# msaelices/mojo-regex

Hardware: AMD Instinct MI355X
Metric: GB/s input scanned + matches/sec, 1M x 1KiB batch, [a-z]+\d+ DFA (higher is better)
Workload: dtype u8

## Files before the change

### include/mrx_testing.h

```cpp
#ifndef MRX_TESTING_H
#define MRX_TESTING_H

#include <stddef.h>
#include <stdint.h>

#ifdef __cplusplus
extern "C" {
#endif

void mrx_timing_reset(void);
void mrx_timing_enable(int on);
double mrx_timing_scan_ms(int64_t* launches);
const char* mrx_last_kernel_name(void);
void mrx_debug_force_generic(int on);
void mrx_debug_long_text_kernels(int mode);
void mrx_debug_fused_findall(int mode);
void mrx_debug_stream_bits(int on);
void mrx_debug_stream_bits_trace(int64_t* d_trace);
void mrx_debug_dynamic_texts(int mode);
void mrx_debug_split_findall(int on);
void mrx_debug_dense_rows(int mode);
void mrx_debug_tries_always(int on);
void mrx_debug_chain_sub_general(int on);
int mrx_testing_emptywalk_findall(const mrx_handle* h, const uint8_t* text, int len, int32_t* spans, int cap);
void mrx_debug_subs_group(int lanes);
void mrx_debug_litscan_pieces(int mode);
void mrx_debug_multiwalk(int mode);
void mrx_debug_rec_skew(int64_t bytes);
void mrx_debug_rec12(int mode);
int mrx_testing_rec12_roundtrip(int start, int pair, int lane, int before, int32_t out[4]);
void mrx_debug_decode_lean(int mode);
int mrx_debug_last_decode_lean(void);
int mrx_testing_decode_expand(int64_t n, const uint32_t* f_even, const uint32_t* f_odd, const int32_t* start, const int32_t* pb,
                              int fixed_len, int32_t* counts, int32_t* spans);
int mrx_testing_comm_shift(const int64_t* d_prefix, int64_t n_local, const int64_t* d_meta_all, int meta_stride, int rank,
                           int64_t* d_out, int64_t pad_to, void* stream);
int mrx_testing_comm_compact(const int64_t* d_meta_all, int meta_stride, int nranks, const int64_t* d_stage_prefix, int64_t P,
                             const int32_t* d_stage_spans, int64_t cap, int64_t* d_gprefix, int64_t gprefix_cap,
                             int32_t* d_gspans, int64_t gspans_cap, int32_t* d_status, void* stream);
void mrx_debug_set_route(int mode);
struct mrx_set;
int mrx_testing_set_run(const struct mrx_set* s, int op, const uint8_t* text, int len, int32_t* out);
void mrx_debug_filter_form(int form);
void mrx_debug_extract_grid(int workgroups);
void mrx_debug_expand_grid(int workgroups);
void mrx_debug_distinct_hash_mask(uint64_t mask);
void mrx_debug_distinct_grid(int workgroups);
void mrx_debug_sort_small(int max);
void mrx_debug_sort_grid(int workgroups);
int mrx_debug_sort_rounds(void);
void mrx_debug_parse_grid(int workgroups);
void mrx_debug_format_grid(int workgroups);
int mrx_testing_format_one(int32_t kind, int32_t arg, int64_t value_word, uint8_t out[32]);
void mrx_debug_kw_piece(int64_t bytes);
void mrx_debug_kw_tier(int on);
int mrx_debug_kw_host_findall(const uint8_t* entry_data, const int64_t* entry_offsets, int64_t m, uint32_t flags,
                              const uint8_t* data, const int64_t* offsets, int64_t n, int64_t* text_prefix, int32_t* entries,
                              int32_t* spans, int64_t span_cap, int64_t* total, char* describe, size_t describe_cap);
int mrx_debug_kw_host_leftmost(const uint8_t* entry_data, const int64_t* entry_offsets, int64_t m, uint32_t flags, int64_t count,
                               const uint8_t* data, const int64_t* offsets, int64_t n, int64_t* text_prefix, int32_t* entries,
                               int32_t* spans, int64_t span_cap, int64_t* total);
int mrx_debug_kw_host_sub(const uint8_t* entry_data, const int64_t* entry_offsets, int64_t m, uint32_t flags,
                          const uint8_t* repl_data, const int64_t* repl_offsets, int64_t r, int64_t count, const uint8_t* data,
                          const int64_t* offsets, int64_t n, int64_t* out_offsets, uint8_t* out_data, int64_t out_cap,
                          int32_t* nsub, int64_t* totals);
// ... 24 lines not shown
```

### mojo_regex_amd/api.py

```python
from __future__ import annotations

import ctypes as C
import os
from typing import Iterable, List, Optional, Sequence, Tuple

import numpy as np

_HERE = os.path.dirname(os.path.abspath(__file__))
_LIB_NAME = "libmrx_hip.so"
_lib = None

MRX_OK, MRX_E_SYNTAX, MRX_E_UNSUPPORTED, MRX_E_NO_DEVICE, MRX_E_CAPACITY, MRX_E_ARGUMENT = range(6)


class MrxError(RuntimeError):
    """Any failure reported by libmrx_hip.so."""


class RegexSyntaxError(MrxError):
    """The reference's lexer/parser raises on this pattern (same message)."""


class UnsupportedPattern(MrxError):
    """The reference routes this pattern/operation to an engine outside the hot
# ... 74 lines not shown
        "mrx_split_batch": (C.c_int, [H, u8p, i64p, C.c_int64, C.c_int64, i64p, i32p, C.c_int64, C.POINTER(C.c_int64)]),
        "mrx_split_dev": (C.c_int, [H, C.c_void_p, C.c_void_p, C.c_int64, C.c_int64, C.c_void_p, C.c_void_p, C.c_int64,
                                    C.POINTER(C.c_int64), C.c_void_p]),
        "mrx_split_strided_dev": (C.c_int, [H, C.c_void_p, C.c_int64, C.c_void_p, C.c_int32, C.c_int64, C.c_int64, C.c_void_p,
                                            C.c_void_p, C.c_int64, C.POINTER(C.c_int64), C.c_void_p]),
        "mrx_findall_batch": (C.c_int, [H, u8p, i64p, C.c_int64, i64p, i32p, C.c_int64,
                                        C.POINTER(C.c_int64)]),
        "mrx_captures_batch": (C.c_int, [H, u8p, i64p, C.c_int64, i32p]),
        "mrx_sub_batch": (C.c_int, [H, C.c_char_p, C.c_size_t, C.c_int64, u8p, i64p, C.c_int64, i64p,
                                    u8p, C.c_int64, C.POINTER(C.c_int64)]),
        "mrx_timing_reset": (None, []),
        "mrx_timing_enable": (None, [C.c_int]),
        "mrx_timing_scan_ms": (C.c_double, [C.POINTER(C.c_int64)]),
        "mrx_last_kernel_name": (C.c_char_p, []),
        "mrx_debug_force_generic": (None, [C.c_int]),
        "mrx_debug_long_text_kernels": (None, [C.c_int]),
        "mrx_debug_fused_findall": (None, [C.c_int]),
        "mrx_debug_stream_bits": (None, [C.c_int]),
        "mrx_debug_stream_bits_trace": (None, [C.c_void_p]),
        "mrx_debug_dynamic_texts": (None, [C.c_int]),
        "mrx_debug_subs_group": (None, [C.c_int]),
        "mrx_debug_split_findall": (None, [C.c_int]),
        "mrx_debug_dense_rows": (None, [C.c_int]),
        "mrx_debug_tries_always": (None, [C.c_int]),
        "mrx_debug_chain_sub_general": (None, [C.c_int]),
        "mrx_testing_emptywalk_findall": (C.c_int, [H, C.c_char_p, C.c_int, i32p, C.c_int]),
        "mrx_debug_litscan_pieces": (None, [C.c_int]),
        "mrx_debug_multiwalk": (None, [C.c_int]),
        "mrx_debug_rec_skew": (None, [C.c_int64]),
        "mrx_debug_rec12": (None, [C.c_int]),
        "mrx_testing_rec12_roundtrip": (C.c_int, [C.c_int, C.c_int, C.c_int, C.c_int, C.POINTER(C.c_int32)]),
        "mrx_debug_decode_lean": (None, [C.c_int]),
        "mrx_debug_last_decode_lean": (C.c_int, []),
        "mrx_testing_decode_expand": (C.c_int, [C.c_int64, C.c_void_p, C.c_void_p, C.c_void_p, C.c_void_p, C.c_int,
                                                C.c_void_p, C.c_void_p]),
        "mrx_release_scratch": (None, []),
        "mrx_debug_scratch_bytes": (C.c_size_t, []),
        "mrx_debug_scratch_in_use": (C.c_size_t, []),
        "mrx_version": (C.c_char_p, []),
        "mrx_comm_unique_id": (C.c_int, [C.c_void_p]),
        "mrx_comm_init": (C.c_int, [C.c_void_p, C.c_int, C.c_int, C.POINTER(H)]),
        "mrx_comm_free": (None, [H]),
        "mrx_comm_rank": (C.c_int, [H]),
        "mrx_comm_size": (C.c_int, [H]),
        "mrx_comm_spans_staging_bytes": (C.c_size_t, [H, C.c_int64, C.c_int64]),
        "mrx_comm_reserve": (C.c_int, [H, C.c_size_t]),
        "mrx_allgather_fixed": (C.c_int, [H, C.c_void_p, C.c_void_p, C.c_size_t, C.c_void_p]),
        "mrx_allgatherv_rows": (C.c_int, [H, C.c_void_p, C.c_int64, C.c_size_t, C.c_void_p, C.c_int64,
                                          C.POINTER(C.c_int64), C.c_void_p]),
        "mrx_allgatherv_spans": (C.c_int, [H, i64p, C.c_int64, i32p, C.c_int64, C.c_int64, i64p, C.c_int64, i32p,
                                           C.c_int64, C.POINTER(C.c_int64), C.POINTER(C.c_int64), i32p, C.c_void_p]),
        "mrx_testing_comm_shift": (C.c_int, [i64p, C.c_int64, i64p, C.c_int, C.c_int, i64p, C.c_int64, C.c_void_p]),
        "mrx_testing_comm_compact": (C.c_int, [i64p, C.c_int, C.c_int, i64p, C.c_int64, i32p, C.c_int64, i64p, C.c_int64,
                                               i32p, C.c_int64, i32p, C.c_void_p]),
        "mrx_set_compile": (C.c_int, [C.POINTER(C.c_char_p), C.POINTER(C.c_size_t), C.c_int32, C.c_uint32, C.POINTER(H)]),
        "mrx_set_free": (None, [H]),
        "mrx_set_size": (C.c_int32, [H]),
        "mrx_set_describe": (C.c_size_t, [H, C.c_char_p, C.c_size_t]),
        "mrx_set_search_dev": (C.c_int, [H, u8p, i64p, C.c_int64, i32p, i32p, C.c_void_p]),
        "mrx_set_search_strided_dev": (C.c_int, [H, u8p, C.c_int64, i32p, C.c_int32, C.c_int64, i32p, i32p, C.c_void_p]),
        "mrx_set_count_dev": (C.c_int, [H, u8p, i64p, C.c_int64, i32p, C.c_void_p]),
        "mrx_set_count_strided_dev": (C.c_int, [H, u8p, C.c_int64, i32p, C.c_int32, C.c_int64, i32p, C.c_void_p]),
        "mrx_set_matches_dev": (C.c_int, [H, u8p, i64p, C.c_int64, i64p, C.c_void_p]),
        "mrx_set_matches_strided_dev": (C.c_int, [H, u8p, C.c_int64, i32p, C.c_int32, C.c_int64, i64p, C.c_void_p]),
        "mrx_set_findall_dev": (C.c_int, [H, u8p, i64p, C.c_int64, i64p, i32p, i32p, C.c_int64, C.POINTER(C.c_int64),
                                          C.c_void_p]),
# ... 225 lines not shown
    "mrx_gather_spans_dev", "mrx_gather_spans_strided_dev", "mrx_gather_spans_batch",
    "mrx_extract_dev", "mrx_extract_known_dev", "mrx_extract_strided_dev", "mrx_extract_batch",
    "mrx_expand_spans_dev", "mrx_expand_spans_strided_dev", "mrx_expand_spans_batch",
    "mrx_expand_dev", "mrx_expand_strided_dev", "mrx_expand_batch",
    "mrx_distinct_dev", "mrx_distinct_known_dev", "mrx_distinct_strided_dev", "mrx_distinct_batch",
    "mrx_dict_build_dev", "mrx_dict_build_strided_dev", "mrx_dict_free", "mrx_dict_size", "mrx_dict_distinct",
    "mrx_dict_lookup_dev", "mrx_dict_lookup_strided_dev", "mrx_dict_filter_dev", "mrx_dict_filter_known_dev",
    "mrx_dict_filter_strided_dev", "mrx_dict_lookup_batch",
    "mrx_sort_dev", "mrx_sort_known_dev", "mrx_sort_strided_dev", "mrx_sort_batch",
    "mrx_take_dev", "mrx_take_known_dev", "mrx_take_strided_dev", "mrx_take_batch",
    "mrx_parse_dev", "mrx_parse_strided_dev", "mrx_parse_spans_dev", "mrx_parse_spans_strided_dev", "mrx_parse_batch",
    "mrx_format_dev", "mrx_format_batch",
    "mrx_kw_build", "mrx_kw_build_dev", "mrx_kw_free", "mrx_kw_size", "mrx_kw_distinct", "mrx_kw_describe",
    "mrx_kw_contains_dev", "mrx_kw_contains_strided_dev", "mrx_kw_count_dev", "mrx_kw_count_strided_dev",
    "mrx_kw_findall_dev", "mrx_kw_findall_known_dev", "mrx_kw_findall_strided_dev", "mrx_kw_filter_dev",
    "mrx_kw_filter_known_dev", "mrx_kw_filter_strided_dev", "mrx_kw_findall_batch",
    "mrx_kw_leftmost_dev", "mrx_kw_leftmost_known_dev", "mrx_kw_leftmost_strided_dev", "mrx_kw_leftmost_batch",
    "mrx_kw_sub_dev", "mrx_kw_sub_known_dev", "mrx_kw_sub_strided_dev", "mrx_kw_sub_batch",
    "mrx_lines_dev", "mrx_lines_known_dev", "mrx_lines_strided_dev", "mrx_lines_batch",
    "mrx_fields_dev", "mrx_fields_known_dev", "mrx_fields_strided_dev", "mrx_fields_batch",
    "mrx_translate_dev", "mrx_translate_known_dev", "mrx_translate_strided_dev", "mrx_translate_batch",
    "mrx_strip_dev", "mrx_strip_known_dev", "mrx_strip_strided_dev", "mrx_strip_batch",
]
TESTING_SYMBOLS = [
    "mrx_timing_reset", "mrx_timing_enable", "mrx_timing_scan_ms", "mrx_last_kernel_name",
    "mrx_debug_force_generic", "mrx_debug_long_text_kernels", "mrx_debug_scratch_bytes",
    "mrx_debug_scratch_in_use",
    "mrx_debug_fused_findall", "mrx_debug_stream_bits", "mrx_debug_stream_bits_trace", "mrx_debug_dynamic_texts", "mrx_debug_subs_group",
    "mrx_debug_split_findall", "mrx_debug_dense_rows", "mrx_debug_tries_always", "mrx_debug_chain_sub_general", "mrx_testing_emptywalk_findall", "mrx_debug_litscan_pieces", "mrx_debug_multiwalk", "mrx_debug_rec_skew", "mrx_testing_comm_shift", "mrx_testing_comm_compact",
    "mrx_debug_set_route", "mrx_testing_set_run", "mrx_debug_filter_form", "mrx_debug_extract_grid",
    "mrx_debug_expand_grid", "mrx_debug_distinct_hash_mask", "mrx_debug_distinct_grid",
    "mrx_debug_sort_small", "mrx_debug_sort_grid", "mrx_debug_sort_rounds", "mrx_debug_parse_grid",
    "mrx_debug_decode_lean", "mrx_debug_last_decode_lean", "mrx_testing_decode_expand",
    "mrx_debug_format_grid", "mrx_testing_format_one",
    "mrx_debug_kw_piece", "mrx_debug_kw_tier", "mrx_debug_kw_host_findall",
    "mrx_debug_kw_host_leftmost", "mrx_debug_kw_host_sub",
    "mrx_debug_lines_piece", "mrx_debug_lines_syncs", "mrx_debug_lines_host",
    "mrx_debug_fields_group", "mrx_debug_fields_grid", "mrx_debug_fields_host",
    "mrx_debug_translate_piece", "mrx_debug_translate_syncs", "mrx_debug_translate_host",
    "mrx_debug_strip_host",
]
TESTING_SYMBOLS_NUMBERED = ["mrx_debug_rec12", "mrx_testing_rec12_roundtrip"]
COMM_SYMBOLS = [
    "mrx_comm_unique_id", "mrx_comm_init", "mrx_comm_free", "mrx_comm_rank", "mrx_comm_size",
    "mrx_comm_spans_staging_bytes", "mrx_comm_reserve",
    "mrx_allgather_fixed", "mrx_allgatherv_rows", "mrx_allgatherv_spans",
]


def _b(x) -> bytes:
    if isinstance(x, str):
        return x.encode("utf-8")
    return bytes(x)


def _check(rc: int):
    if rc == MRX_OK:
        return
    msg = load_library().mrx_last_error().decode("utf-8", "replace")
    if rc == MRX_E_SYNTAX:
        raise RegexSyntaxError(msg)
    if rc == MRX_E_UNSUPPORTED:
        raise UnsupportedPattern(msg)
    raise MrxError("mrx error %d: %s" % (rc, msg))


# ... 1897 lines not shown
```

### mojo_regex_amd/csrc/mrx_kernels.hip

```cpp
#include <hip/hip_runtime.h>
#include <atomic>
#include <map>
#include <type_traits>
#include <unordered_map>
#include <chrono>

#include <cstdio>
#include <cstdlib>
#include <cstring>
#include <mutex>
#include <string>
#include <vector>

#include "../../include/mrx.h"
#include "../../include/mrx_testing.h"
#include "mrx_device.hpp"
#include "mrx_host_batch.hpp"
#include "mrx_internal.hpp"
#include "mrx_lookback.hpp"
#include "mrx_rec12.hpp"
#include "mrx_decode_bits.hpp"

using namespace mrx;

namespace {

constexpr int kBlock = 256;

struct Layout : TextBatch {
  Layout() = default;
  Layout(const TextBatch& b) : TextBatch(b) {}
  int32_t split = 0;
  int32_t wide_slots = 0;
  const int32_t* vlen = nullptr;
  const uint32_t* vskip = nullptr;
  const int32_t* vbase = nullptr;
  const int2* pre = nullptr;
  const uint32_t* bm = nullptr;
  const int32_t* bm_cnt = nullptr;
  __host__ __device__ __forceinline__ int64_t bm_row(int64_t i) const {
    return 4 * (offsets ? (offsets[i] >> 7) + 2 * i : i * ((stride >> 7) + 2));
  }
  __device__ __forceinline__ int64_t slot_row(int64_t i, int* cap) const {
    if (offsets) {
// ... 1573 lines not shown
    base = fused_lookback(fz.ctrl, w, nw, lane);
    if (base < 0) {
    } else
    if (total_spans > 3 * tile_cap) {
      fused_fill_tile<REC32, true>(wave_recs, wrec, my_rel, 0, base, tile, tile_bytes, fz.spans, fz.span_cap, fixed_len, lane);
    } else {
      for (int tb = 0; tb < total_spans; tb += tile_cap) {
        fused_fill_tile<REC32, false>(wave_recs, wrec, my_rel, tb, 0, tile, tile_bytes, fz.spans, fz.span_cap, fixed_len, lane);
        fused_store_tile<REC32>(tile, total_spans - tb < tile_cap ? total_spans - tb : tile_cap, base + tb, fz.spans,
                                fz.span_cap, lane);
      }
    }
  }
  const int64_t my_text = (w << 6) + lane;
  if (base < 0) {
    if (lane == 0) { fz.prefix[n] = -1; *fz.total_out = -1; }
    return;
  }
  if (my_text < n) fz.prefix[my_text] = base + my_rel;
  if (my_text == n - 1) { fz.prefix[n] = base + incl; *fz.total_out = base + incl; }
}

template <int MODE, int CH, int AUTO, int CSR, int VIRT = 0, int REC32 = 0>
#ifndef MRX_FUSED_WAVES
#define MRX_FUSED_WAVES 4
#endif
__global__ __launch_bounds__(64 * kStreamWaves, (MODE == ST_FUSED ? MRX_FUSED_WAVES : 1)) void k_stream_findall(
    DevPlan p, const uint8_t* __restrict__ blob, const uint8_t* __restrict__ data, int64_t stride,
    const int32_t* __restrict__ lens, int32_t common_len, const int64_t* __restrict__ offsets,
    int64_t n, int32_t* __restrict__ counts,
    int32_t* __restrict__ wave_nrecs, EvRec* __restrict__ recs, int64_t rec_row,
    int32_t* __restrict__ out_s, int32_t* __restrict__ out_e,
    const int32_t* __restrict__ vlen = nullptr, const uint32_t* __restrict__ vskip = nullptr,
    const FusedArgs* __restrict__ fzp = nullptr) {
#define fz (*fzp)
  constexpr bool RECS = MODE == ST_RECORDS || MODE == ST_FUSED;
  constexpr bool ROWS = MODE == ST_ROWS;
  static_assert(!(MODE == ST_FUSED && VIRT), "pieces of long texts keep the three-launch form");
  static_assert(!ROWS || (!CSR && !VIRT && !REC32), "event rows: texts at a fixed aligned pitch");
  constexpr bool REC12 = REC32 == 2;
  static_assert(!REC12 || (MODE == ST_RECORDS && !CSR && !VIRT), "12-byte records: the three-launch form at a fixed aligned pitch");
  constexpr int kChunk = CH;
  constexpr int kRowPitch = CH + 16;
  constexpr int LPR = CH / 16;
  constexpr int RPI = 64 / LPR;
  constexpr int NL = 64 / RPI;
  __shared__ __align__(16) uint8_t tiles[kStreamWaves][64 * kRowPitch];
  __shared__ __align__(16) uint16_t col_lds[256];
  __shared__ __align__(16) uint16_t col32_lds[AUTO == 5 ? 256 : 2];
  static_assert(AUTO != 5 || MODE != ST_FIRST, "the anchored automaton has no code-column form");
  __shared__ __align__(16) uint4 pmask[17];
  if (threadIdx.x < 17) {
    const int x = threadIdx.x;
    uint32_t w[4];
    for (int j = 0; j < 4; ++j) {
      const int nb = x - 4 * j;
      w[j] = nb <= 0 ? 0u : nb >= 4 ? 0xFFFFFFFFu : ((1u << (8 * nb)) - 1u);
    }
    pmask[x] = make_uint4(w[0], w[1], w[2], w[3]);
  }
  __shared__ unsigned long long blk_ticket[4];
  if (MODE == ST_FUSED && threadIdx.x == 0) {
    blk_ticket[1] = blk_ticket[2] = blk_ticket[3] = 0ull;
    blk_ticket[0] = (1ull << 32) | (uint32_t)__hip_atomic_fetch_add(fz.ctrl, (unsigned long long)kStreamWaves, __ATOMIC_RELAXED,
                                                                    __HIP_MEMORY_SCOPE_AGENT);
  }
  const bool use_fill = AUTO == 5 || (MODE != ST_FIRST && p.st_reset_byte >= 0 && !(MODE == ST_COUNT && (AUTO == 2 || AUTO == 3)));
  const uint32_t fillw = (uint32_t)(p.st_reset_byte & 0xFF) * 0x01010101u;
  extern __shared__ __align__(16) uint8_t stg_lds[];
  if (AUTO == 5) {
    const uint16_t* src = (const uint16_t*)(blob + p.off_stcol32);
    for (int i = threadIdx.x; i < 256; i += blockDim.x) col32_lds[i] = src[i];
  } else if (AUTO == 1) {
    const uint16_t* src = (const uint16_t*)(blob + (MODE == ST_FIRST ? p.off_fa_col : p.off_stcol));
    for (int i = threadIdx.x; i < 256; i += blockDim.x) col_lds[i] = src[i];
  } else if (AUTO == 3) {
    const uint32_t* src = (const uint32_t*)(blob + (MODE == ST_FIRST ? p.off_fa_col : p.off_stcol));
    uint32_t* dst = (uint32_t*)stg_lds;
    for (int i = threadIdx.x; i < 512; i += blockDim.x) dst[i] = src[i];
  } else {
    const uint32_t* src = (const uint32_t*)(blob + (MODE == ST_FIRST ? p.off_fa_cls : p.off_stg_cls));
    uint32_t* dst = (uint32_t*)stg_lds;
    const int words = (MODE == ST_FIRST ? p.fa_bytes : p.stg_bytes) >> 2;
    for (int i = threadIdx.x; i < words; i += blockDim.x) dst[i] = src[i];
  }
  __syncthreads();
  const uint64_t* col64_lds = (const uint64_t*)stg_lds;
  const uint8_t* cls_lds = stg_lds;
  const uint16_t* tr_lds = (const uint16_t*)(stg_lds + (MODE == ST_FIRST ? p.off_fa_trans - p.off_fa_cls
                                                                        : p.off_stg_trans - p.off_stg_cls));
  const uint8_t* acc_lds = stg_lds + (p.off_stg_acc - p.off_stg_cls);
  const uint32_t* pair_lds = (const uint32_t*)(stg_lds + (p.off_stg_pair - p.off_stg_cls));
  const uint32_t fa_dead = AUTO == 2 ? (uint32_t)p.fa_nstates << p.fa_cshift
                                     : (uint32_t)p.fa_nstates * (AUTO == 1 ? 4u : 8u);
  const int lane = threadIdx.x & 63;
  const int wave = threadIdx.x >> 6;
  uint8_t* tile = tiles[wave];
  const int64_t nwaves_total = (n + 63) >> 6;
  const uint32_t accmask = p.st_accept_mask;
  const int seg = lane % LPR;
  const int rsub = lane / LPR;

  unsigned long long tk_next = 0ull;
  bool tk_asked = false;
  uint32_t round = 0;
  bool pend = false;
  int64_t pend_w = 0;
  int pend_cnt = 0, pend_wrec = 0, pend_half = 0, half = 0;
  for (int64_t w = (int64_t)blockIdx.x * kStreamWaves + wave;; w += (int64_t)gridDim.x * kStreamWaves) {
    if (MODE == ST_FUSED) {
      unsigned long long tv;
      while (true) {
        tv = *(volatile unsigned long long*)&blk_ticket[round & 3u];
        if ((uint32_t)(tv >> 32) == round + 1u) break;
        __builtin_amdgcn_s_sleep(1);
      }
      const int64_t first = (int64_t)__builtin_amdgcn_readfirstlane((uint32_t)tv);
      w = first + wave;
      tk_asked = wave == 0 && first < nwaves_total;
      if (tk_asked) {
        if (lane == 0)
          tk_next = __hip_atomic_fetch_add(fz.ctrl, (unsigned long long)kStreamWaves, __ATOMIC_RELAXED, __HIP_MEMORY_SCOPE_AGENT);
        asm volatile("" ::: "memory");
      } else if (wave == 0 && lane == 0) {
        blk_ticket[(round + 1u) & 3u] = ((unsigned long long)(round + 2u) << 32) | (uint32_t)nwaves_total;
      }
      ++round;
    }
    if (w >= nwaves_total) break;
    const int64_t base_text = w << 6;
    const int64_t my_text = base_text + lane;
    const bool live = my_text < n;
    int my_len, mis = 0;
    if (CSR) {
      int64_t o0;
      if (offsets) {
        o0 = live ? offsets[my_text] : 0;
        my_len = live ? (VIRT ? vlen[my_text] : (int)(offsets[my_text + 1] - o0)) : 0;
      } else {
        o0 = my_text * stride;
        my_len = live ? (lens ? lens[my_text] : common_len) : 0;
      }
      const uintptr_t addr = my_len > 0 ? (uintptr_t)(data + o0) : (uintptr_t)blob;
      constexpr uintptr_t kFrameMask = MODE == ST_FIRST ? 15 : 127;
      mis = my_len > 0 ? (int)(addr & kFrameMask) : 0;
      const uintptr_t rb = addr & ~kFrameMask;
      *(uint4*)(tile + lane * kRowPitch + CH) =
          make_uint4((uint32_t)rb, (uint32_t)((uint64_t)rb >> 32), (uint32_t)(mis + my_len), 0u);
      __builtin_amdgcn_fence(__ATOMIC_RELEASE, "wavefront");
      __builtin_amdgcn_wave_barrier();
      __builtin_amdgcn_fence(__ATOMIC_ACQUIRE, "wavefront");
    } else {
      my_len = live ? (lens ? lens[my_text] : common_len) : 0;
    }
    const uint32_t vsk = (VIRT && live) ? vskip[my_text] : 0u;
    const int skip = (int)(vsk & 0x7FFFFFFFu);
    const int flen = mis + my_len;
    int max_len = flen;
    for (int off = 32; off > 0; off >>= 1) max_len = max(max_len, __shfl_xor(max_len, off));

    const uint8_t* wbase = data + base_text * stride;
    const int64_t rows_here = n - base_text < 64 ? n - base_text : 64;
    uint32_t roff[NL];
#pragma unroll
    for (int j = 0; j < NL; ++j) {
      int r = RPI * j + rsub;
      if (r >= rows_here) r = (int)rows_here - 1;
      roff[j] = (uint32_t)(r * stride) + seg * 16;
    }
#define MRX_LOAD_CHUNK(CB)                                                       \
    do {                                                                         \
      uint32_t cb_ = (uint32_t)(CB);                                             \
      if (!CSR && (int64_t)cb_ + seg * 16 >= stride) cb_ = (uint32_t)0 - (uint32_t)(seg * 16); \
      _Pragma("unroll") for (int j_ = 0; j_ < NL; ++j_)                          \
        if (MODE != ST_FIRST || !((skip_rows >> (RPI * j_ + rsub)) & 1ull)) {     \
          if (CSR) {                                                             \
            const uint4 rs_ = *(const uint4*)(tile + (RPI * j_ + rsub) * kRowPitch + CH); \
            uint32_t fo_ = cb_ + seg * 16;                                       \
            if (fo_ >= rs_.z) fo_ = 0;   \
            v[j_] = MRX_LDG((const uint4*)((const uint8_t*)(((uint64_t)rs_.y << 32) | rs_.x) + fo_)); \
          } else {                                                               \
            v[j_] = MRX_LDG((const uint4*)(wbase + (roff[j_] + cb_)));                   \
          }                                                                      \
        }                                                                        \
    } while (0)
    uint64_t skip_rows = 0;

    uint32_t q4 = 0;
    uint32_t q_codes = 0;
    int start = 0;
    int cnt = 0;
    int wrec = 0;
    bool done = !live;
    int res_s = -1, res_e = (MODE == ST_FIRST && live && p.fa_start_acc) ? 0 : -1;
    EvRec* wave_recs = (MODE == ST_RECORDS)
        ? recs + ((CSR && offsets) ? rec_region_start(offsets[base_text], w) : base_text * rec_row)
        : (MODE == ST_FUSED) ? recs + (((int64_t)blockIdx.x * kStreamWaves + wave) * 2 + half) * fz.rec_cap : nullptr;
    uint32_t* const wave_recs12 = REC12 ? (uint32_t*)recs + 3 * (base_text * rec_row) : nullptr;

    if (MODE == ST_FIRST) {
      uint4 pv = make_uint4(0, 0, 0, 0);
      if (live && my_len > 0) {
        if (CSR) pv = *(const uint4*)(((uintptr_t)(data + (offsets ? offsets[my_text] : my_text * stride))) & ~(uintptr_t)15);
        else pv = *(const uint4*)(data + my_text * stride);
      }
      const uint32_t pw[4] = {pv.x, pv.y, pv.z, pv.w};
      uint32_t pq = 0, pF = 0;
#pragma unroll
      for (int k = 0; k < 16; ++k) {
        const uint32_t b = (pw[k >> 2] >> ((k & 3) * 8)) & 0xFFu;
        const bool outside = k < mis || k >= flen;
        uint32_t e;
        if (AUTO == 2) {
          e = tr_lds[pq + cls_lds[b]];
          if (outside) e = pq << 2;
          pq = e >> 2;
        } else if (AUTO == 1) {
          e = (uint32_t)col_lds[b] >> pq;
          if (outside) e = pq;
          pq = e & 0xCu;
        } else {
          e = (uint32_t)(col64_lds[b] >> pq);
          if (outside) e = pq;
          pq = e & 0x38u;
        }
        pF = __builtin_amdgcn_alignbit(e, pF, 2);
      }
      const uint32_t pem = pF & 0xAAAAAAAAu;
      if (__all(!live || pq == fa_dead || flen <= 16)) {
        if (live) {
          int e_ = pem ? ((31 - __builtin_clz(pem)) >> 1) + 1 - mis : (p.fa_start_acc ? 0 : -1);
          if (AUTO == 2 && p.off_fa_end >= 0 && stg_lds[(p.off_fa_end - p.off_fa_cls) + (pq >> p.fa_cshift)]) e_ = my_len;
          out_s[my_text] = e_ >= 0 ? 0 : -1;
          out_e[my_text] = e_;
        }
        continue;
      }
    }
    uint4 v[NL];
#pragma unroll
    for (int j = 0; j < NL; ++j) v[j] = make_uint4(0, 0, 0, 0);
    if (max_len > 0) MRX_LOAD_CHUNK(0);
    uint8_t* wr = tile + rsub * kRowPitch + seg * 16;
    uint4 rowacc[ROWS ? 8 : 1];
    for (int cbase = 0; cbase < max_len; cbase += kChunk) {
#pragma unroll
      for (int j = 0; j < NL; ++j) *(uint4*)(wr + j * RPI * kRowPitch) = v[j];
      __builtin_amdgcn_fence(__ATOMIC_RELEASE, "wavefront");
      __builtin_amdgcn_wave_barrier();
      __builtin_amdgcn_fence(__ATOMIC_ACQUIRE, "wavefront");
      if (MODE == ST_SEARCH) { if (__all(done)) break; }
      if (MODE == ST_FIRST) {
        skip_rows = __ballot(done || cbase + kChunk >= flen);
        if (__all(done)) break;
      }
      if (MODE == ST_FUSED && tk_asked) {
        const uint32_t nf = __builtin_amdgcn_readfirstlane((uint32_t)tk_next);
        if (lane == 0) blk_ticket[round & 3u] = ((unsigned long long)(round + 1u) << 32) | nf;
        tk_asked = false;
      }
      if (!(MRX_ABLATE & 2))
      if (cbase + kChunk < max_len) MRX_LOAD_CHUNK(cbase + kChunk);

      const int lim = flen - cbase;
      const int lo = mis - cbase;
      const bool all_inside = __all(lim >= kChunk && lo <= 0);
      const bool full = all_inside || use_fill;
      uint32_t F_even = 0, meta_even = 0, sp_even = 0;
      uint2 rowbuf[ROWS ? kChunk / 32 : 1];
#pragma unroll
      for (int g = 0; g < kChunk / 16; ++g) {
        const uint4 wv = *(const uint4*)(tile + lane * kRowPitch + g * 16);
        uint32_t words[4] = {wv.x, wv.y, wv.z, wv.w};
        if (use_fill && !all_inside) {
          const int limf = (VIRT && !(vsk >> 31)) ? 0x3FFFFFFF : lim;
          const int a = min(max(lo - g * 16, 0), 16), b = min(max(limf - g * 16, 0), 16);
          const uint4 pa = pmask[a], pb = pmask[b > a ? b : a];
          const uint32_t m[4] = {pb.x & ~pa.x, pb.y & ~pa.y, pb.z & ~pa.z, pb.w & ~pa.w};
#pragma unroll
          for (int j = 0; j < 4; ++j) words[j] = (words[j] & m[j]) | (fillw & ~m[j]);
        }
        uint32_t F = 0;
        if (AUTO == 4) {
          uint32_t cc[16], pi[8];
#pragma unroll
          for (int k = 0; k < 16; ++k)
            cc[k] = cls_lds[(words[k >> 2] >> ((k & 3) * 8)) & 0xFFu];
#pragma unroll
          for (int k = 0; k < 8; ++k) pi[k] = (cc[2 * k] << p.st_cshift) | cc[2 * k + 1];
#pragma unroll
          for (int k = 0; k < 8; ++k) {
            const uint32_t e = pair_lds[q4 + pi[k]];
            q4 = e >> 4;
            F = __builtin_amdgcn_alignbit(e, F, 4);
          }
// ... 189 lines not shown
        for (int off = 32; off > 0; off >>= 1) wt += __shfl_xor(wt, off);
        if (lane == 0) wave_nrecs[nwaves_total + w] = wt;
      }
      if (MODE == ST_FIRST) {
        if (live) {
          if (AUTO == 2 && p.off_fa_end >= 0 && stg_lds[(p.off_fa_end - p.off_fa_cls) + (q4 >> p.fa_cshift)]) res_e = my_len;
          out_s[my_text] = res_e >= 0 ? 0 : -1;
          out_e[my_text] = res_e;
        }
      } else if (MODE == ST_SEARCH) {
        if (live) {
          if (!done && tail) { res_s = p.st_fixed_len > 0 ? my_len - p.st_fixed_len : start; res_e = my_len; }
          out_s[my_text] = res_s;
          out_e[my_text] = res_e;
        }
      } else if (MODE == ST_FUSED) {
        int wt = live ? cnt : 0;
        for (int off = 32; off > 0; off >>= 1) wt += __shfl_xor(wt, off);
        fused_publish(fz.ctrl, w, nwaves_total, (uint32_t)wt, lane);
        if (pend)
          fused_finish<REC32 != 0>(fz, recs + (((int64_t)blockIdx.x * kStreamWaves + wave) * 2 + pend_half) * fz.rec_cap,
                                   pend_w, nwaves_total, n, pend_cnt, pend_wrec, tile, 64 * kRowPitch, p.st_fixed_len, lane);
        pend = true; pend_w = w; pend_cnt = live ? cnt : 0; pend_wrec = wrec; pend_half = half;
        half ^= 1;
      } else {
        if (live) counts[my_text] = cnt;
      }
    }
  }
  if (MODE == ST_FUSED && pend)
    fused_finish<REC32 != 0>(fz, recs + (((int64_t)blockIdx.x * kStreamWaves + wave) * 2 + pend_half) * fz.rec_cap,
                             pend_w, nwaves_total, n, pend_cnt, pend_wrec, tile, 64 * kRowPitch, p.st_fixed_len, lane);
#undef MRX_LOAD_CHUNK
#undef fz
}

#ifndef MRX_DYN_TEXTS
#define MRX_DYN_TEXTS 256
#endif
constexpr int kDynTexts = MRX_DYN_TEXTS;
constexpr int kDynShift = kDynTexts <= 256 ? 24 : kDynTexts <= 512 ? 23 : 22;
constexpr uint32_t kDynBeforeMask = (1u << kDynShift) - 1u;
static_assert(kDynTexts % 64 == 0 && kDynTexts <= 1024, "task size");
__host__ __device__ inline int64_t rec_region_dyn(int64_t first_off, int64_t w) { return (first_off >> 4) + 4 * kDynTexts * w; }

template <int MODE, int AUTO, int REC32>
__global__ __launch_bounds__(64 * kStreamWaves) void k_stream_dyn(
    DevPlan p, const uint8_t* __restrict__ blob, const uint8_t* __restrict__ data, const int64_t* __restrict__ offsets,
    const int32_t* __restrict__ vlen, int64_t n, int32_t* __restrict__ counts, int32_t* __restrict__ wave_nrecs,
    EvRec* __restrict__ recs, int32_t* __restrict__ out_s, int32_t* __restrict__ out_e) {
  static_assert(MODE == ST_RECORDS || MODE == ST_COUNT || MODE == ST_SEARCH, "search modes only");
#ifndef MRX_DYN_CH
#define MRX_DYN_CH 128
#endif
  constexpr int CH = MRX_DYN_CH, kRowPitch = CH + 16, LPR = CH / 16, RPI = 64 / LPR, NL = 64 / RPI;
  __shared__ __align__(16) uint8_t tiles[kStreamWaves][64 * kRowPitch];
  __shared__ __align__(16) uint16_t col_lds[256];
  __shared__ __align__(16) uint4 pmask[17];
  __shared__ uint16_t perm_all[kStreamWaves][kDynTexts];
  __shared__ int hist_all[kStreamWaves][32];
  if (threadIdx.x < 17) {
    const int x = threadIdx.x;
    uint32_t w[4];
    for (int j = 0; j < 4; ++j) {
      const int nb = x - 4 * j;
      w[j] = nb <= 0 ? 0u : nb >= 4 ? 0xFFFFFFFFu : ((1u << (8 * nb)) - 1u);
// ... 2237 lines not shown
  }
  HIP_TRY(hipGetLastError());
  tm.stop();
  return MRX_OK;
}

std::atomic<int> g_fused{0};
std::atomic<int64_t> g_rec_skew{0};
std::atomic<int> g_fused_bpc{0};
int64_t fused_grid_cap() {
  const int bpc = g_fused_bpc.load() > 0 ? g_fused_bpc.load() : 4;
  return (int64_t)(grid_cap() / 8) * bpc;
}
constexpr int64_t kFusedMinTaskBytes = 32768;
bool anchored_at_zero(const mrx_handle* h) {
  const DevPlan& p = h->hp.dev;
  return !g_force_generic && (p.flags & PF_START_ANCHOR) && !(p.flags & PF_PURE_LITERAL) &&
         (!(p.flags & PF_END_ANCHOR) || p.off_fa_end >= 0) &&
         p.kind == PLAN_DFA && p.fa_bytes > 0 && !(p.flags & (PF_EXACT_LITERAL | PF_PREFILTER)) && h->hp.why_no_search.empty();
}
constexpr int64_t kStreamMaxText = int64_t(1) << 26;
bool stream_text_too_long(int64_t max_text) { return max_text >= kStreamMaxText; }
bool stream_layout_ok(const Layout&, int64_t n) { return n > 0; }
bool strided_fast(const Layout& lay) {
  return !lay.offsets && (lay.stride % 16 == 0) && (((uintptr_t)lay.data) % 16 == 0) &&
         lay.stride * 64 < (int64_t(1) << 31);
}

static bool code_columns_on() {
  static const bool on = [] { const char* e = getenv("MRX_NO_CODE_COLUMNS"); return !(e && e[0] == '1'); }();
  return on;
}

template <int MODE>
void launch_stream(const mrx_handle* h, const Layout& lay, int64_t n, int32_t* d_counts, int32_t* d_nrecs,
                   EvRec* d_recs, int64_t rec_row, int32_t* d_s, int32_t* d_e, hipStream_t s,
                   const int32_t* d_vlen = nullptr, const uint32_t* d_vskip = nullptr, int rec32 = 0,
                   const FusedArgs* fused = nullptr, int fused_grid = 0) {
  const DevPlan& p = h->hp.dev;
  const int g = MODE == ST_FUSED ? fused_grid : wave_grid(n, kStreamWaves);
  const FusedArgs* fzv = fused;
  const dim3 grid((unsigned)g), block(64 * kStreamWaves);
  const int kind = MODE == ST_FIRST ? p.fa_kind : p.st_kind;
  const bool table = kind == 2;
  const bool wide = kind == 3;
  const bool pairs = MODE != ST_FIRST && (table || wide) && p.off_stg_pair >= 0 && g_pair_tables;
  const size_t lds = pairs ? (size_t)p.stg_bytes
                           : wide ? 2048 : !table ? 0 : (size_t)(MODE == ST_FIRST ? p.fa_bytes : p.stg_bytes);
#define MRX_LAUNCH_R(AUTO, CSR, R32)                                                              \
  hipLaunchKernelGGL((k_stream_findall<MODE, (AUTO == 2 ? MRX_STREAM_CHUNK_TABLE : MRX_STREAM_CHUNK), AUTO, CSR, 0, R32>), grid, block, lds, s, p, \
                     H_BLOB(h), lay.data, lay.stride, lay.lens, lay.len, lay.offsets, n, d_counts, \
                     d_nrecs, d_recs, rec_row, d_s, d_e, (const int32_t*)nullptr, (const uint32_t*)nullptr, fzv)
#define MRX_LAUNCH(AUTO, CSR)                                                                     \
  do {                                                                                            \
    if constexpr (MODE == ST_RECORDS && CSR == 0) {                                               \
      if (rec32 == 2) { MRX_LAUNCH_R(AUTO, CSR, 2); break; }                                      \
    }                                                                                             \
    if constexpr (MODE == ST_RECORDS || MODE == ST_FUSED) {                                       \
      if (rec32) MRX_LAUNCH_R(AUTO, CSR, 1); else MRX_LAUNCH_R(AUTO, CSR, 0);                     \
    } else MRX_LAUNCH_R(AUTO, CSR, 0);                                                            \
  } while (0)
  if (d_vlen) {
    if constexpr (MODE == ST_RECORDS || MODE == ST_COUNT || MODE == ST_SEARCH || MODE == ST_FIRST) {
#define MRX_LAUNCH_V(AUTO)                                                                        \
  hipLaunchKernelGGL((k_stream_findall<MODE, (AUTO == 2 ? MRX_STREAM_CHUNK_TABLE : MRX_STREAM_CHUNK), AUTO, 1, 1>), grid, block, lds, s, p, \
                     H_BLOB(h), lay.data, lay.stride, lay.lens, lay.len, lay.offsets, n, d_counts, \
                     d_nrecs, d_recs, rec_row, d_s, d_e, d_vlen, d_vskip)
      if (pairs) { if constexpr (MODE != ST_FIRST) MRX_LAUNCH_V(4); }
      else if (table) MRX_LAUNCH_V(2);
      else if (wide) MRX_LAUNCH_V(3);
      else MRX_LAUNCH_V(1);
#undef MRX_LAUNCH_V
    }
  } else if (!strided_fast(lay)) {
    if constexpr (MODE != ST_ROWS) {
    if (pairs) { if constexpr (MODE != ST_FIRST) MRX_LAUNCH(4, 1); }
    else if (table) MRX_LAUNCH(2, 1);
    else if (wide) MRX_LAUNCH(3, 1);
    else MRX_LAUNCH(1, 1);
    }
  } else {
    if (pairs) { if constexpr (MODE != ST_FIRST) MRX_LAUNCH(4, 0); }
    else if (table) MRX_LAUNCH(2, 0);
    else if (wide) MRX_LAUNCH(3, 0);
    else if (MODE != ST_FIRST && MODE != ST_COUNT && p.off_stcol32 >= 0 && code_columns_on()) { if constexpr (MODE != ST_FIRST && MODE != ST_COUNT) MRX_LAUNCH(5, 0); }
// ... 2666 lines not shown
  HIP_TRY(hipMemcpy(spans, sp.p, sizeof(int32_t) * per * n, hipMemcpyDeviceToHost));
  return MRX_OK;
}
int mrx_sub_batch(const mrx_handle* h, const char* repl, size_t repl_len, int64_t count,
                  const uint8_t* data, const int64_t* off, int64_t n, int64_t* out_offsets,
                  uint8_t* out_data, int64_t out_cap, int64_t* total_bytes) {
  DevBatch b; DevBuf<int64_t> oo; DevBuf<uint8_t> od;
  if (int rc = b.upload(data, off, n)) return rc;
  if (int rc = oo.alloc(n + 1)) return rc;
  if (int rc = od.alloc((size_t)out_cap)) return rc;
  int64_t tot = 0;
  const int rc = mrx_sub_dev(h, repl, repl_len, count, b.data, b.offsets, n, oo.p, od.p, out_cap,
                             &tot, nullptr);
  if (total_bytes) *total_bytes = tot;
  if (rc != MRX_OK && rc != MRX_E_CAPACITY) return rc;
  HIP_TRY(hipMemcpy(out_offsets, oo.p, sizeof(int64_t) * (n + 1), hipMemcpyDeviceToHost));
  if (rc == MRX_OK && tot > 0) HIP_TRY(hipMemcpy(out_data, od.p, (size_t)tot, hipMemcpyDeviceToHost));
  return rc;
}

void mrx_timing_reset(void) { g_scan_ms = 0; g_scan_launches = 0; }
void mrx_timing_enable(int on) { g_timing = on != 0; }
double mrx_timing_scan_ms(int64_t* launches) {
  if (launches) *launches = g_scan_launches;
  return g_scan_launches ? g_scan_ms / (double)g_scan_launches : 0.0;
}
const char* mrx_last_kernel_name(void) { return g_last_kernel; }
void mrx_debug_force_generic(int on) { g_force_generic = on < 0 ? 0 : on > 2 ? 2 : on; }
void mrx_debug_long_text_kernels(int mode) { g_long_text_mode = mode < 0 ? 0 : mode > 3 ? 0 : mode; }
void mrx_debug_rec_skew(int64_t bytes) { g_rec_skew = bytes < 0 ? 0 : (bytes & ~int64_t(15)); }
void mrx_debug_rec12(int mode) { g_rec12 = mode != 0; }
void mrx_debug_decode_lean(int mode) { g_decode_lean = mode != 0; }
int mrx_debug_last_decode_lean(void) { return g_last_decode_lean; }
int mrx_testing_decode_expand(int64_t n, const uint32_t* f_even, const uint32_t* f_odd, const int32_t* start, const int32_t* pb,
                              int fixed_len, int32_t* counts, int32_t* spans) {
  if (n < 0 || fixed_len < 0 || (n > 0 && (!f_even || !f_odd || !start || !pb || !counts || !spans))) return -1;
  for (int64_t i = 0; i < n; ++i) {
    int32_t* out = spans + 64 * i;
    int cnt = 0;
    auto emit = [&](int st, int end) { out[2 * cnt] = st; out[2 * cnt + 1] = end; ++cnt; };
    if (fixed_len > 0) decode_expand_record<true>(f_even[i], f_odd[i], start[i], pb[i], fixed_len, emit);
    else decode_expand_record<false>(f_even[i], f_odd[i], start[i], pb[i], fixed_len, emit);
    counts[i] = cnt;
  }
  return 0;
}
int mrx_testing_rec12_roundtrip(int start, int pair, int lane, int before, int32_t out[4]) {
  if (start < 0 || start >= kRec12MaxLen || pair < 0 || pair > kRec12MaxLen / 32 || lane < 0 || lane > 63 || before < 0 ||
      before >= kRec12MaxLen || !out)
    return -1;
  const uint32_t m = rec12_pack((uint32_t)start, (uint32_t)pair, (uint32_t)lane, (uint32_t)before);
  out[0] = rec12_start(m); out[1] = rec12_pair(m); out[2] = rec12_lane(m); out[3] = rec12_before(m);
  return 0;
}
void mrx_debug_fused_findall(int mode) { g_fused = mode < 0 ? 0 : mode > 2 ? 0 : mode; }
void mrx_debug_stream_bits(int on) { mrx::stream_bits_set_mode(on); }
void mrx_debug_stream_bits_trace(int64_t* d_trace) { mrx::stream_bits_set_trace(d_trace); }
void mrx_debug_dynamic_texts(int mode) { g_dyn_mode = mode < 0 ? 0 : mode > 2 ? 0 : mode; }
void mrx_debug_split_findall(int on) { g_split_findall = on ? 1 : 0; }
void mrx_debug_dense_rows(int mode) { g_dense_rows = mode; }
void mrx_debug_tries_always(int on) { g_tries_always = on ? 1 : 0; }
void mrx_debug_chain_sub_general(int on) { g_chain_sub_general = on ? 1 : 0; }
int mrx_testing_emptywalk_findall(const mrx_handle* h, const uint8_t* text, int len, int32_t* spans, int cap) {
  if (!h || !h->hp.ew2_ok || len < 0) return -1;
  const std::vector<std::pair<int, int>> v = emptywalk2_run(h->hp.ew2, text, len);
  for (size_t k = 0; k < v.size() && (int)k < cap; ++k) { spans[2 * k] = v[k].first; spans[2 * k + 1] = v[k].second; }
// ... 67 lines not shown
```

Baseline: 3792.

## Add persistent-grid stream scan with cross-task prefetch of next wave's first chunk

Adds an optional persistent-grid mode for the records/count stream scan. The grid is sized to the number of resident workgroups from an occupancy query, and each wave prefetches the lengths and first data chunk of its next text group during the last chunk of the current one. The goal is to hide load latency between grid-stride iterations and cut launch tail effects. The mode is off by default (MRX_SCAN_PERSIST=0), but the kernel still gains an extra parameter, uses readfirstlane for the wave index, and hoists the data array v out of the loop, which may raise register pressure.

```diff
diff --git a/include/mrx_testing.h b/include/mrx_testing.h
--- a/include/mrx_testing.h
+++ b/include/mrx_testing.h
@@ -31,6 +31,8 @@
 int mrx_testing_rec12_roundtrip(int start, int pair, int lane, int before, int32_t out[4]);
 void mrx_debug_decode_lean(int mode);
 int mrx_debug_last_decode_lean(void);
+void mrx_debug_scan_persist(int mode);
+void mrx_debug_scan_grid(int workgroups);
 int mrx_testing_decode_expand(int64_t n, const uint32_t* f_even, const uint32_t* f_odd, const int32_t* start, const int32_t* pb,
                               int fixed_len, int32_t* counts, int32_t* spans);
 int mrx_testing_comm_shift(const int64_t* d_prefix, int64_t n_local, const int64_t* d_meta_all, int meta_stride, int rank,
diff --git a/mojo_regex_amd/api.py b/mojo_regex_amd/api.py
--- a/mojo_regex_amd/api.py
+++ b/mojo_regex_amd/api.py
@@ -130,6 +130,8 @@
         "mrx_testing_rec12_roundtrip": (C.c_int, [C.c_int, C.c_int, C.c_int, C.c_int, C.POINTER(C.c_int32)]),
         "mrx_debug_decode_lean": (None, [C.c_int]),
         "mrx_debug_last_decode_lean": (C.c_int, []),
+        "mrx_debug_scan_persist": (None, [C.c_int]),
+        "mrx_debug_scan_grid": (None, [C.c_int]),
         "mrx_testing_decode_expand": (C.c_int, [C.c_int64, C.c_void_p, C.c_void_p, C.c_void_p, C.c_void_p, C.c_int,
                                                 C.c_void_p, C.c_void_p]),
         "mrx_release_scratch": (None, []),
@@ -421,6 +423,7 @@
     "mrx_debug_expand_grid", "mrx_debug_distinct_hash_mask", "mrx_debug_distinct_grid",
     "mrx_debug_sort_small", "mrx_debug_sort_grid", "mrx_debug_sort_rounds", "mrx_debug_parse_grid",
     "mrx_debug_decode_lean", "mrx_debug_last_decode_lean", "mrx_testing_decode_expand",
+    "mrx_debug_scan_persist", "mrx_debug_scan_grid",
     "mrx_debug_format_grid", "mrx_testing_format_one",
     "mrx_debug_kw_piece", "mrx_debug_kw_tier", "mrx_debug_kw_host_findall",
     "mrx_debug_kw_host_leftmost", "mrx_debug_kw_host_sub",
diff --git a/mojo_regex_amd/csrc/mrx_kernels.hip b/mojo_regex_amd/csrc/mrx_kernels.hip
--- a/mojo_regex_amd/csrc/mrx_kernels.hip
+++ b/mojo_regex_amd/csrc/mrx_kernels.hip
@@ -10,6 +10,7 @@
 #include <cstring>
 #include <mutex>
 #include <string>
+#include <tuple>
 #include <vector>
 
 #include "../../include/mrx.h"
@@ -1649,10 +1650,11 @@
     int32_t* __restrict__ wave_nrecs, EvRec* __restrict__ recs, int64_t rec_row,
     int32_t* __restrict__ out_s, int32_t* __restrict__ out_e,
     const int32_t* __restrict__ vlen = nullptr, const uint32_t* __restrict__ vskip = nullptr,
-    const FusedArgs* __restrict__ fzp = nullptr) {
+    const FusedArgs* __restrict__ fzp = nullptr, int32_t xtask = 0) {
 #define fz (*fzp)
   constexpr bool RECS = MODE == ST_RECORDS || MODE == ST_FUSED;
   constexpr bool ROWS = MODE == ST_ROWS;
+  constexpr bool XT = !CSR && !VIRT && (MODE == ST_RECORDS || MODE == ST_COUNT);
   static_assert(!(MODE == ST_FUSED && VIRT), "pieces of long texts keep the three-launch form");
   static_assert(!ROWS || (!CSR && !VIRT && !REC32), "event rows: texts at a fixed aligned pitch");
   constexpr bool REC12 = REC32 == 2;
@@ -1711,7 +1713,7 @@
   const uint32_t fa_dead = AUTO == 2 ? (uint32_t)p.fa_nstates << p.fa_cshift
                                      : (uint32_t)p.fa_nstates * (AUTO == 1 ? 4u : 8u);
   const int lane = threadIdx.x & 63;
-  const int wave = threadIdx.x >> 6;
+  const int wave = XT ? __builtin_amdgcn_readfirstlane(threadIdx.x >> 6) : threadIdx.x >> 6;
   uint8_t* tile = tiles[wave];
   const int64_t nwaves_total = (n + 63) >> 6;
   const uint32_t accmask = p.st_accept_mask;
@@ -1724,6 +1726,10 @@
   bool pend = false;
   int64_t pend_w = 0;
   int pend_cnt = 0, pend_wrec = 0, pend_half = 0, half = 0;
+  bool have_nx = false;
+  bool pre = false;
+  int nx_len = 0;
+  uint4 v[NL];
   for (int64_t w = (int64_t)blockIdx.x * kStreamWaves + wave;; w += (int64_t)gridDim.x * kStreamWaves) {
     if (MODE == ST_FUSED) {
       unsigned long long tv;
@@ -1767,25 +1773,38 @@
       __builtin_amdgcn_fence(__ATOMIC_RELEASE, "wavefront");
       __builtin_amdgcn_wave_barrier();
       __builtin_amdgcn_fence(__ATOMIC_ACQUIRE, "wavefront");
+    } else if (XT && have_nx) {
+      my_len = nx_len;
     } else {
       my_len = live ? (lens ? lens[my_text] : common_len) : 0;
     }
+    const int64_t wn = w + (int64_t)gridDim.x * kStreamWaves;
+    const bool has_next = XT && xtask != 0 && wn < nwaves_total;
     const uint32_t vsk = (VIRT && live) ? vskip[my_text] : 0u;
     const int skip = (int)(vsk & 0x7FFFFFFFu);
     const int flen = mis + my_len;
     int max_len = flen;
     for (int off = 32; off > 0; off >>= 1) max_len = max(max_len, __shfl_xor(max_len, off));
+    if (XT) {
+      have_nx = has_next;
+      if (has_next) {
+        const int64_t nt = (wn << 6) + lane;
+        nx_len = nt < n ? (lens ? lens[nt] : common_len) : 0;
+      }
+    }
 
     const uint8_t* wbase = data + base_text * stride;
     const int64_t rows_here = n - base_text < 64 ? n - base_text : 64;
-    uint32_t roff[NL];
-#pragma unroll
-    for (int j = 0; j < NL; ++j) {
-      int r = RPI * j + rsub;
-      if (r >= rows_here) r = (int)rows_here - 1;
-      roff[j] = (uint32_t)(r * stride) + seg * 16;
-    }
-#define MRX_LOAD_CHUNK(CB)                                                       \
+    uint32_t roff[XT ? 1 : NL];
+    if (!XT) {
+#pragma unroll
+      for (int j = 0; j < (XT ? 1 : NL); ++j) {
+        int r = RPI * j + rsub;
+        if (r >= rows_here) r = (int)rows_here - 1;
+        roff[j] = (uint32_t)(r * stride) + seg * 16;
+      }
+    }
+#define MRX_LOAD_CHUNK_AT(BASE, ROWS, CB)                                        \
     do {                                                                         \
       uint32_t cb_ = (uint32_t)(CB);                                             \
       if (!CSR && (int64_t)cb_ + seg * 16 >= stride) cb_ = (uint32_t)0 - (uint32_t)(seg * 16); \
@@ -1796,11 +1815,15 @@
             uint32_t fo_ = cb_ + seg * 16;                                       \
             if (fo_ >= rs_.z) fo_ = 0;   \
             v[j_] = MRX_LDG((const uint4*)((const uint8_t*)(((uint64_t)rs_.y << 32) | rs_.x) + fo_)); \
+          } else if (XT) {                                                       \
+            const uint32_t ro_ = (uint32_t)min(RPI * j_ + rsub, (int)(ROWS) - 1) * (uint32_t)stride + seg * 16; \
+            v[j_] = MRX_LDG((const uint4*)((BASE) + (ro_ + cb_)));               \
           } else {                                                               \
-            v[j_] = MRX_LDG((const uint4*)(wbase + (roff[j_] + cb_)));                   \
+            v[j_] = MRX_LDG((const uint4*)(wbase + (roff[XT ? 0 : j_] + cb_)));  \
           }                                                                      \
         }                                                                        \
     } while (0)
+#define MRX_LOAD_CHUNK(CB) MRX_LOAD_CHUNK_AT(wbase, rows_here, CB)
     uint64_t skip_rows = 0;
 
     uint32_t q4 = 0;
@@ -1854,10 +1877,12 @@
         continue;
       }
     }
-    uint4 v[NL];
-#pragma unroll
-    for (int j = 0; j < NL; ++j) v[j] = make_uint4(0, 0, 0, 0);
-    if (max_len > 0) MRX_LOAD_CHUNK(0);
+    if (!(XT && pre)) {
+#pragma unroll
+      for (int j = 0; j < NL; ++j) v[j] = make_uint4(0, 0, 0, 0);
+      if (max_len > 0) MRX_LOAD_CHUNK(0);
+    }
+    pre = false;
     uint8_t* wr = tile + rsub * kRowPitch + seg * 16;
     uint4 rowacc[ROWS ? 8 : 1];
     for (int cbase = 0; cbase < max_len; cbase += kChunk) {
@@ -1876,8 +1901,17 @@
         if (lane == 0) blk_ticket[round & 3u] = ((unsigned long long)(round + 1u) << 32) | nf;
         tk_asked = false;
       }
-      if (!(MRX_ABLATE & 2))
-      if (cbase + kChunk < max_len) MRX_LOAD_CHUNK(cbase + kChunk);
+      if (!(MRX_ABLATE & 2)) {
+        if (cbase + kChunk < max_len) {
+          MRX_LOAD_CHUNK(cbase + kChunk);
+        } else if (XT && has_next) {
+          const int64_t nx_base = wn << 6;
+          int nx_max = nx_len;
+          for (int off = 32; off > 0; off >>= 1) nx_max = max(nx_max, __shfl_xor(nx_max, off));
+          if (nx_max > 0) MRX_LOAD_CHUNK_AT(data + nx_base * stride, (n - nx_base < 64 ? n - nx_base : 64), 0);
+          pre = true;
+        }
+      }
 
       const int lim = flen - cbase;
       const int lo = mis - cbase;
@@ -2133,6 +2167,7 @@
     fused_finish<REC32 != 0>(fz, recs + (((int64_t)blockIdx.x * kStreamWaves + wave) * 2 + pend_half) * fz.rec_cap,
                              pend_w, nwaves_total, n, pend_cnt, pend_wrec, tile, 64 * kRowPitch, p.st_fixed_len, lane);
 #undef MRX_LOAD_CHUNK
+#undef MRX_LOAD_CHUNK_AT
 #undef fz
 }
 
@@ -4436,6 +4471,31 @@
   return on;
 }
 
+static int env_int(const char* name, int dflt);
+std::atomic<int> g_scan_persist{env_int("MRX_SCAN_PERSIST", 0)};
+std::atomic<int> g_scan_grid{0};
+static int stream_resident(const void* fn, size_t lds) {
+  static std::mutex mu;
+  static std::map<std::tuple<const void*, size_t, int>, int> known;
+  std::lock_guard<std::mutex> lock(mu);
+  const auto key = std::make_tuple(fn, lds, t_dev);
+  const auto it = known.find(key);
+  if (it != known.end()) return it->second;
+  int per_cu = 0;
+  if (hipOccupancyMaxActiveBlocksPerMultiprocessor(&per_cu, fn, 64 * kStreamWaves, lds) != hipSuccess || per_cu < 0) per_cu = 0;
+  const int g = per_cu * (grid_cap() / 8);
+  known[key] = g;
+  return g;
+}
+static int persist_grid(const void* fn, size_t lds, int64_t n, int parent_grid) {
+  const int64_t wgs = ((n + 63) / 64 + kStreamWaves - 1) / kStreamWaves;
+  const int res = stream_resident(fn, lds);
+  int64_t g = res > 0 ? (wgs < res ? wgs : res) : parent_grid;
+  const int cap = g_scan_grid.load(std::memory_order_relaxed);
+  if (cap > 0 && g > cap) g = cap;
+  return (int)(g < 1 ? 1 : g);
+}
+
 template <int MODE>
 void launch_stream(const mrx_handle* h, const Layout& lay, int64_t n, int32_t* d_counts, int32_t* d_nrecs,
                    EvRec* d_recs, int64_t rec_row, int32_t* d_s, int32_t* d_e, hipStream_t s,
@@ -4452,9 +4512,21 @@
   const size_t lds = pairs ? (size_t)p.stg_bytes
                            : wide ? 2048 : !table ? 0 : (size_t)(MODE == ST_FIRST ? p.fa_bytes : p.stg_bytes);
 #define MRX_LAUNCH_R(AUTO, CSR, R32)                                                              \
-  hipLaunchKernelGGL((k_stream_findall<MODE, (AUTO == 2 ? MRX_STREAM_CHUNK_TABLE : MRX_STREAM_CHUNK), AUTO, CSR, 0, R32>), grid, block, lds, s, p, \
-                     H_BLOB(h), lay.data, lay.stride, lay.lens, lay.len, lay.offsets, n, d_counts, \
-                     d_nrecs, d_recs, rec_row, d_s, d_e, (const int32_t*)nullptr, (const uint32_t*)nullptr, fzv)
+  do {                                                                                            \
+    const auto kfn_ = k_stream_findall<MODE, (AUTO == 2 ? MRX_STREAM_CHUNK_TABLE : MRX_STREAM_CHUNK), AUTO, CSR, 0, R32>; \
+    dim3 grid_ = grid;                                                                            \
+    int32_t xtask_ = 0;                                                                           \
+    if constexpr ((MODE == ST_RECORDS || MODE == ST_COUNT) && CSR == 0) {                         \
+      const int pm_ = g_scan_persist.load(std::memory_order_relaxed);                             \
+      if (pm_) {                                        \
+        if (pm_ != 2) grid_.x = (unsigned)persist_grid((const void*)kfn_, lds, n, g);             \
+        xtask_ = pm_ != 3;                                                                        \
+      }                                                                                           \
+    }                                                                                             \
+    hipLaunchKernelGGL(kfn_, grid_, block, lds, s, p,                                             \
+                       H_BLOB(h), lay.data, lay.stride, lay.lens, lay.len, lay.offsets, n, d_counts, \
+                       d_nrecs, d_recs, rec_row, d_s, d_e, (const int32_t*)nullptr, (const uint32_t*)nullptr, fzv, xtask_); \
+  } while (0)
 #define MRX_LAUNCH(AUTO, CSR)                                                                     \
   do {                                                                                            \
     if constexpr (MODE == ST_RECORDS && CSR == 0) {                                               \
@@ -7187,6 +7259,8 @@
 void mrx_debug_rec12(int mode) { g_rec12 = mode != 0; }
 void mrx_debug_decode_lean(int mode) { g_decode_lean = mode != 0; }
 int mrx_debug_last_decode_lean(void) { return g_last_decode_lean; }
+void mrx_debug_scan_persist(int mode) { g_scan_persist = mode < 0 || mode > 3 ? 1 : mode; }
+void mrx_debug_scan_grid(int workgroups) { g_scan_grid = workgroups > 0 ? workgroups : 0; }
 int mrx_testing_decode_expand(int64_t n, const uint32_t* f_even, const uint32_t* f_odd, const int32_t* start, const int32_t* pb,
                               int fixed_len, int32_t* counts, int32_t* spans) {
   if (n < 0 || fixed_len < 0 || (n > 0 && (!f_even || !f_odd || !start || !pb || !counts || !spans))) return -1;
```

Result: slower. 3591 (-5.3%).
